# open-flash/swf-renderer

Measured on AMD Instinct MI355X. Metric: Mpixels/sec rasterized @ 4K, 10k-edge synthetic shape set, higher is better.
Workload: dtype i32+f64(exact integers)/u8

## Files before the change

### swf_renderer_amd/csrc/device_types.hpp

```cpp
#pragma once

#include <stdint.h>

#include "../../include/swfr.h"

namespace swfr {

constexpr int TILE_W = 64;
constexpr int TILE_H = 16;
constexpr int STRIP_H = 8;
constexpr int STRIPS_PER_TILE = TILE_H / STRIP_H;

struct DevEdge {
    int32_t ytop, ybot;
    int32_t x1, y1;
    int32_t dir;
    int32_t pad;
    int64_t ex;
    int64_t dy;
    int64_t dq, dr;
    double inv_dy;
    double inv_dx;
    int64_t fr;
    int64_t r15;
// ... 124 lines not shown
struct StripDesc {
    uint32_t wg;
    uint32_t band_begin, n_b;
    uint32_t pad;
};

struct StripTop {
    uint32_t any, pad;
    unsigned long long cover;
};
static_assert(sizeof(StripTop) == 16, "StripTop layout");

constexpr uint32_t XCDS = 8;
inline uint32_t strip_slots(uint32_t local_tile_rows, uint32_t strips_per_row) { return XCDS * ((local_tile_rows + XCDS - 1) / XCDS) * strips_per_row; }
constexpr uint32_t BIN_THREADS_LARGE = 1024, BIN_THREADS_SMALL = 256, BIN_SMALL_PATHS = 16 * BIN_THREADS_SMALL;

struct Frame2 {
    const swfr_edge* raw; const DevPath* paths;
    const swfr_style* styles;
    Sources src;
    const uint32_t* path_chunks; const uint32_t* path_slots; const uint32_t* path_inc;
    const uint32_t* band_off;
    const uint32_t* path_bands;
    ChunkInfo* chunks; BandSlot* band_slots; StripDesc* strips;
    uint32_t* strip_cost;
    DevEdge* edges; BandEntry2* band_list; uint8_t* cls; RowInfo2* rows; Cell* cells; SlowRow* slow; SlowRow* huge; uint32_t* counters;
    uint32_t* path_flag; uint32_t* path_queue;
    uint32_t* fb;
    StripTop* strip_top;
    uint32_t n_edges, n_paths, n_chunks, n_bands, n_strips, cell_slice, slow_cap;
// ... 17 lines not shown
```

### swf_renderer_amd/csrc/frame_layout.hpp

```cpp
#pragma once
#include <stddef.h>
#include <stdint.h>

#include "device_types.hpp"

namespace swfr {

inline size_t pad256(size_t bytes) { return (bytes + 255) & ~size_t(255); }

struct FrameDims {
    size_t n_edges = 0, n_paths = 0, n_slots = 0, n_rows = 0, n_chunks = 0, n_strips = 0, n_strip_slots = 0, cell_total = 0;
    template <class Layout>
    static FrameDims of_layout(const Layout& L, size_t n_edges, size_t n_paths) {
        return FrameDims{n_edges, n_paths, L.n_slots, L.n_rows, L.n_chunks, L.n_strips, L.n_strip_slots, L.cell_total};
    }

    size_t edge_count() const { return 2 * n_edges + 1; }
    size_t band_entry_count() const { return n_slots; }
    size_t row_count() const { return n_slots * TILE_H + 64; }
    size_t cell_count() const { return cell_total; }
    size_t slow_count() const { return 2 * (n_rows + 64); }
    size_t path_word_count() const { return n_paths + 64; }
    size_t chunk_count() const { return n_chunks + 1; }
    size_t band_slot_count() const { return n_slots + 8; }
    size_t strip_count() const { return n_strip_slots + 1; }
    size_t strip_cost_count() const { return n_strips + 1; }
};

template <class V>
void for_each_frame_buffer(Frame2& f, const FrameDims& d, V&& v) {
    v(f.edges, d.edge_count()); v(f.band_list, d.band_entry_count()); v(f.rows, d.row_count()); v(f.cells, d.cell_count());
    v(f.slow, d.slow_count()); v(f.huge, d.slow_count()); v(f.path_flag, d.path_word_count()); v(f.path_queue, d.path_word_count());
    v(f.chunks, d.chunk_count()); v(f.band_slots, d.band_slot_count()); v(f.strips, d.strip_count()); v(f.strip_cost, d.strip_cost_count());
    v(f.counters, size_t(C2_WORDS));
}
inline uint8_t* carve_frame(Frame2& f, const FrameDims& d, uint8_t* base) {
    for_each_frame_buffer(f, d, [&](auto*& p, size_t n) { p = reinterpret_cast<decltype(p + 0)>(base); base += pad256(n * sizeof(*p)); });
    return base;
}
inline size_t frame_work_bytes(const FrameDims& d) {
    Frame2 f{};
    size_t bytes = 0;
    for_each_frame_buffer(f, d, [&](auto* p, size_t n) { bytes += pad256(n * sizeof(*p)); });
    return bytes;
}

inline size_t cls_bytes_of(size_t n_slots, size_t tiles_x) { return (size_t(STRIPS_PER_TILE) * n_slots * tiles_x + 64 + 15) & ~size_t(15); }
inline size_t cls_region_bytes(size_t n_slots, size_t tiles_x, size_t n_strips) { return cls_bytes_of(n_slots, tiles_x) + (n_strips + 1) * sizeof(StripTop); }
inline size_t cls_region_bytes(const FrameDims& d, size_t tiles_x) { return cls_region_bytes(d.n_slots, tiles_x, d.n_strips); }
inline void set_cls_region(Frame2& f, const FrameDims& d, size_t tiles_x, uint8_t* base) {
    f.cls = base;
    f.strip_top = reinterpret_cast<StripTop*>(base + cls_bytes_of(d.n_slots, tiles_x));
}

}
```

### swf_renderer_amd/csrc/raster2.hip

```cpp
#include "raster_common.hip"

namespace swfr {

__device__ __forceinline__ void lds_barrier() {
#ifdef SWFR_EMU
    __syncthreads();
#else
    __builtin_amdgcn_fence(__ATOMIC_RELEASE, "workgroup", "local");
    __builtin_amdgcn_s_barrier();
    __builtin_amdgcn_fence(__ATOMIC_ACQUIRE, "workgroup", "local");
#endif
}

#ifdef SWFR_EMU
typedef const Frame2* FramePtr;
#define FRAME_PTR(frames, i) ((frames) + (i))
#else
typedef const Frame2 __attribute__((address_space(4)))* FramePtr;
#define FRAME_PTR(frames, i) ((FramePtr)((frames) + (i)))
#endif

#ifdef SWFR_TSTATS
#define TRACE_WGS 32768
__device__ uint32_t swfr_trace_buf[3][TRACE_WGS][8];
// ... 279 lines not shown
        for (uint32_t c = 0; c < nc; ++c) write_chunk(ip, c, a0, c0, inc0, slots0, first_edge, n_path_edges, band0);
    for (unsigned long long big = __ballot(nc > OWN_CHUNKS); big; big &= big - 1ull) {
        const int src = __ffsll((long long)big) - 1;
        const uint32_t b_nc = (uint32_t)__shfl((int)nc, src), b_path = (uint32_t)__shfl((int)ip, src), b_a0 = (uint32_t)__shfl((int)a0, src);
        const uint32_t b_c0 = (uint32_t)__shfl((int)c0, src), b_inc0 = (uint32_t)__shfl((int)inc0, src), b_slots0 = (uint32_t)__shfl((int)slots0, src);
        const uint32_t b_fe = (uint32_t)__shfl((int)first_edge, src), b_ne = (uint32_t)__shfl((int)n_path_edges, src), b_band0 = (uint32_t)__shfl((int)band0, src);
        for (uint32_t c = (uint32_t)lane; c < b_nc; c += 64u) write_chunk(b_path, c, b_a0, b_c0, b_inc0, b_slots0, b_fe, b_ne, b_band0);
    }
}
constexpr uint32_t ORDER_RANGES = 8;
__device__ __forceinline__ uint32_t order_range(uint32_t cost) {
    return cost >= 48u ? 0u : cost >= 32u ? 1u : cost >= 24u ? 2u : cost >= 16u ? 3u : cost >= 8u ? 4u : cost >= 4u ? 5u : cost >= 1u ? 6u : 7u;
}
constexpr uint32_t ORDER_U = 16;
template <uint32_t BIN_THREADS> __device__ __forceinline__ void order_body(FramePtr F, uint32_t x) {
    __shared__ uint2 rowinfo[256];
    __shared__ uint32_t cnt[ORDER_RANGES][ORDER_U][BIN_THREADS / 64];
    const int tid = threadIdx.x, lane = tid & 63, wave = tid >> 6;
    const uint32_t n_strips = F->n_strips, bc = F->band_stride, bi = F->band_first;
    const uint32_t per_row = STRIPS_PER_TILE * (uint32_t)F->tiles_x;
    const uint32_t n_local = n_strips / per_row;
    const uint32_t rows_x = (n_local + XCDS - 1 - x) / XCDS, max_rows = (n_local + XCDS - 1) / XCDS;
    const uint32_t n_mine = rows_x * per_row;
    const bool by_cost = F->strip_order != 0u;
    for (uint32_t j = (uint32_t)tid; j < rows_x && j < 256u; j += BIN_THREADS) {
        const uint32_t trow = (x + j * XCDS) * bc + bi, b0 = F->band_off[trow];
        rowinfo[j] = make_uint2(b0, F->band_off[trow + 1] - b0);
    }
    if (rows_x < max_rows)
        for (uint32_t j = (uint32_t)tid; j < per_row; j += BIN_THREADS) {
            StripDesc sd; sd.wg = ~0u; sd.band_begin = 0; sd.n_b = 0; sd.pad = 0;
            F->strips[(size_t)(n_mine + j) * XCDS + x] = sd;
        }
    __syncthreads();
    const uint32_t dq = BIN_THREADS / per_row, dr = BIN_THREADS - dq * per_row;
    auto advance = [&](uint32_t& j, uint32_t& pos) { j += dq; pos += dr; if (pos >= per_row) { pos -= per_row; ++j; } };
    auto strip_at = [&](uint32_t j, uint32_t pos) { return (x + j * XCDS) * per_row + pos; };
    for (uint32_t base = 0; base < n_mine; base += ORDER_U * BIN_THREADS) {
        const uint32_t n_round = min(n_mine - base, ORDER_U * BIN_THREADS), U = (n_round + BIN_THREADS - 1) / BIN_THREADS;
        unsigned long long ranges = 0;
// ... 42 lines not shown
            }
            __syncthreads();
        } else {
#pragma unroll
            for (uint32_t u = 0; u < ORDER_U; ++u) behind[u] = 0;
        }
        uint32_t j = j0, pos = pos0;
#pragma unroll
        for (uint32_t u = 0; u < ORDER_U; ++u) {
            if (u >= U) continue;
            const uint32_t i = base + u * BIN_THREADS + (uint32_t)tid;
            if (i < n_mine) {
                uint32_t rank = i;
                if (by_cost) rank = base + cnt[(uint32_t)(ranges >> (3 * u)) & 7u][u][wave] + behind[u];
                uint2 ri;
                if (j < 256u) ri = rowinfo[j]; else { const uint32_t trow = (x + j * XCDS) * bc + bi, b0 = F->band_off[trow]; ri = make_uint2(b0, F->band_off[trow + 1] - b0); }
                StripDesc sd; sd.wg = strip_at(j, pos); sd.band_begin = ri.x; sd.n_b = ri.y; sd.pad = (pos / STRIPS_PER_TILE) | ((x + j * XCDS) << 16);
                F->strips[(size_t)rank * XCDS + x] = sd;
            }
            advance(j, pos);
        }
        __syncthreads();
    }
}
__global__ __launch_bounds__(1024) __attribute__((amdgpu_num_sgpr(80))) void k2_bin_b(const Frame2* __restrict__ frames, uint32_t slow_kernels) { TRACE_DECL; TRACE_NOWAIT(0); bin_body<BIN_THREADS_LARGE, BIN_ORDER_FIRST_LARGE != 0>(FRAME_PTR(frames, blockIdx.y), slow_kernels); TRACE(7); TRACE_OUT(0, blockIdx.x); }
__global__ __launch_bounds__(256) void k2_bin_small_b(const Frame2* __restrict__ frames, uint32_t slow_kernels) { TRACE_DECL; TRACE_NOWAIT(0); bin_body<BIN_THREADS_SMALL, BIN_ORDER_FIRST_SMALL != 0>(FRAME_PTR(frames, blockIdx.y), slow_kernels); TRACE(7); TRACE_OUT(0, blockIdx.x); }

__device__ __forceinline__ uint32_t pack_sub_cell(int x, int sgn, int xminp, int xmaxp) {
    int col = x >> 8, f = x & 255, live = 1;
    if (col >= xmaxp) { col = xmaxp - 1; f = 0; live = 0; }
    else if (col < xminp) { col = xminp; f = 0; }
// ... 7 lines not shown
#define R2_WAVES 5
#endif
#define R2_ATTR __attribute__((amdgpu_waves_per_eu(R2_WAVES)))
#ifndef R2_WIDE_WAVES
#define R2_WIDE_WAVES 3
#endif
__global__ __launch_bounds__(64) R2_ATTR void k2_rows_b(const Frame2* __restrict__ frames) {
    FramePtr FR = FRAME_PTR(frames, blockIdx.y);
    if (blockIdx.x >= FR->n_chunks) return;
    rows3_chunk_body<ROWS_STAGE, ROWS_FAST_N>(FR, blockIdx.x);
}
__global__ __launch_bounds__(64) __attribute__((amdgpu_waves_per_eu(R2_WIDE_WAVES))) void k2_rows_wide_b(const Frame2* __restrict__ frames) {
    FramePtr FR = FRAME_PTR(frames, blockIdx.y);
    if (blockIdx.x >= FR->n_chunks) return;
    rows3_chunk_body<ROWS_STAGE_WIDE, ROWS_FAST_WIDE>(FR, blockIdx.x);
}

#include "mono.hip"

__global__ __launch_bounds__(64) void k2_rows_mono_b(const Frame2* __restrict__ frames) {
    FramePtr FR = FRAME_PTR(frames, blockIdx.y);
    if (blockIdx.x >= FR->n_chunks) return;
    mono_chunk_body(FR, blockIdx.x);
}
__global__ __launch_bounds__(HUGE_THREADS) void k2_rows_mono_huge_b(const Frame2* __restrict__ frames) { mono_huge_loop(FRAME_PTR(frames, blockIdx.y)); }


__device__ __forceinline__ void sort_pairs(uint16_t* __restrict__ dst, const int* __restrict__ cell, int p, int cnt) {
    const int x = 2 * p, y = 2 * p + 1;
    if (y < cnt) { const bool keep = cell[x] <= cell[y]; dst[x] = (uint16_t)(keep ? x : y); dst[y] = (uint16_t)(keep ? y : x); }
// ... 1314 lines not shown
#endif
__global__ __launch_bounds__(64) __attribute__((amdgpu_waves_per_eu(T2_WAVES_SHADED))) void k2_tiles_bitmap_b(const Frame2* __restrict__ frames, uint32_t* fb_to) { tiles3_body<1>(FRAME_PTR(frames, blockIdx.y), fb_to); }
__global__ __launch_bounds__(64) __attribute__((amdgpu_waves_per_eu(T2_WAVES_SHADED))) void k2_tiles_shaded_b(const Frame2* __restrict__ frames, uint32_t* fb_to) { tiles3_body<2>(FRAME_PTR(frames, blockIdx.y), fb_to); }
__global__ __launch_bounds__(64) __attribute__((amdgpu_waves_per_eu(T2_WAVES_BLEND))) void k2_tiles_blend_b(const Frame2* __restrict__ frames, uint32_t* fb_to) { tiles3_body<3>(FRAME_PTR(frames, blockIdx.y), fb_to); }
__global__ __launch_bounds__(64) __attribute__((amdgpu_waves_per_eu(T2_WAVES_LAYER))) void k2_tiles_layer_b(const Frame2* __restrict__ frames, uint32_t* fb_to) { tiles3_body<4>(FRAME_PTR(frames, blockIdx.y), fb_to); }
__global__ __launch_bounds__(64) __attribute__((amdgpu_waves_per_eu(T2_WAVES_LAYER))) void k2_tiles_mask_b(const Frame2* __restrict__ frames, uint32_t* fb_to) { tiles3_body<5>(FRAME_PTR(frames, blockIdx.y), fb_to); }
__global__ __launch_bounds__(64) __attribute__((amdgpu_waves_per_eu(T2_WAVES_LAYER))) void k2_tiles_fade_b(const Frame2* __restrict__ frames, uint32_t* fb_to) { tiles3_body<6>(FRAME_PTR(frames, blockIdx.y), fb_to); }
__global__ __launch_bounds__(64) __attribute__((amdgpu_waves_per_eu(T2_WAVES_LAYER))) void k2_tiles_alpha_b(const Frame2* __restrict__ frames, uint32_t* fb_to) { tiles3_body<7>(FRAME_PTR(frames, blockIdx.y), fb_to); }

void launch2_bin(hipStream_t st, const Frame2* frames, uint32_t n_frames, uint32_t max_edges, uint32_t max_paths, uint32_t max_bands, uint32_t slow_kernels, bool mono, uint32_t bin_threads) {
    const uint32_t T = bin_threads == BIN_THREADS_SMALL ? BIN_THREADS_SMALL : BIN_THREADS_LARGE;
    const uint32_t g = XCDS + max_bands + (mono ? 0u : (max_edges + T - 1) / T) + (max_paths + T - 1) / T;
    if (T == BIN_THREADS_SMALL) hipLaunchKernelGGL(k2_bin_small_b, dim3(g, n_frames), dim3(BIN_THREADS_SMALL), 0, st, frames, slow_kernels);
    else hipLaunchKernelGGL(k2_bin_b, dim3(g, n_frames), dim3(BIN_THREADS_LARGE), 0, st, frames, slow_kernels);
}
void launch2_rows(hipStream_t st, const Frame2* frames, uint32_t n_frames, uint32_t max_chunks, uint32_t max_path_edges, bool wide, bool mono) {
    if (!max_chunks) return;
    if (mono) { hipLaunchKernelGGL(k2_rows_mono_b, dim3(max_chunks, n_frames), dim3(64), 0, st, frames); return; }
    if (wide || max_path_edges > ROWS_STAGE) hipLaunchKernelGGL(k2_rows_wide_b, dim3(max_chunks, n_frames), dim3(64), 0, st, frames);
    else hipLaunchKernelGGL(k2_rows_b, dim3(max_chunks, n_frames), dim3(64), 0, st, frames);
}
void launch2_rows_slow(hipStream_t st, const Frame2* frames, uint32_t n_frames, uint32_t grid_slow, uint32_t grid_huge, uint32_t max_passes, bool mono) {
    if (mono) { hipLaunchKernelGGL(k2_rows_mono_huge_b, dim3(grid_huge ? grid_huge : 64u, n_frames), dim3(HUGE_THREADS), 0, st, frames); return; }
    if (grid_slow) hipLaunchKernelGGL(k2_start_ranks_b, dim3(grid_slow / 4 + 1, n_frames), dim3(256), 0, st, frames);
    for (uint32_t pass = 0; pass < SLOW_PASSES; ++pass) {
        if (grid_slow) hipLaunchKernelGGL(k2_rows_slow_b, dim3(grid_slow, n_frames), dim3(64), 0, st, frames, pass);
        if (grid_huge) hipLaunchKernelGGL(k2_rows_huge_b, dim3(grid_huge, n_frames), dim3(HUGE_THREADS), 0, st, frames, pass);
        if (pass + 1 >= max_passes) break;
    }
}
__device__ __forceinline__ void linear_pieces_body(FramePtr FR) {
    if (blockIdx.x >= FR->n_linear_records) return;
    const DevGradient* G = FR->src.gradients + blockIdx.x;
    if (G->pad <= 0) return;
    int32_t* table = const_cast<int32_t*>(FR->src.fparams) + (G->pad - 1);
// ... 85 lines not shown
```

### swf_renderer_amd/csrc/renderer.cpp

```cpp
#include <hip/hip_runtime.h>

#include <algorithm>
#include <chrono>
#include <cfloat>
#include <cmath>
#include <cstdio>
#include <cstdlib>
#include <cstring>
#include <exception>
#include <map>
#include <memory>
#include <stdexcept>
#include <string>
#include <unordered_map>
#include <vector>

#include "../../include/swfr.h"
#include "device_types.hpp"
#include "frame_layout.hpp"
#include "frame_builder.hpp"
#include "shape_decoder.hpp"
#include "bitmap_decode.hpp"

namespace swfr {
void launch2_bin(hipStream_t, const Frame2*, uint32_t, uint32_t, uint32_t, uint32_t, uint32_t, bool, uint32_t);
void launch2_rows(hipStream_t, const Frame2*, uint32_t, uint32_t, uint32_t, bool, bool);
void launch2_rows_slow(hipStream_t, const Frame2*, uint32_t, uint32_t, uint32_t, uint32_t, bool);
void launch2_tiles(hipStream_t, const Frame2*, uint32_t, uint32_t, uint32_t, int, uint32_t*);
void launch2_linear_pieces(hipStream_t, const Frame2*, uint32_t, uint32_t);
void launch_unpremultiply(hipStream_t, const uint32_t*, uint32_t*, size_t);
void launch_pack_band(hipStream_t, const uint32_t*, uint32_t*, int, int, uint32_t, uint32_t, uint32_t);
void launch_cxform_texels(hipStream_t, const uint8_t*, uint32_t*, size_t, const uint32_t*);
void launch_blur_capture(hipStream_t, const uint32_t*, uint32_t*, size_t);
void launch_blur_pass(hipStream_t, const uint32_t*, uint32_t*, uint32_t, uint32_t, uint32_t, bool);
void launch_shadow_alpha(hipStream_t, const uint32_t*, uint32_t*, uint32_t, uint32_t, int32_t, int32_t);
void launch_shadow_finish(hipStream_t, const uint32_t*, const uint32_t*, bool, uint32_t*, size_t, uint32_t, uint32_t, uint32_t);
}

using namespace swfr;

namespace {
// ... 119 lines not shown
    swfr_config cfg{};
    bool has_device = false;
    std::string error;
    std::unique_ptr<FrameBuilder> builder;
    std::string json_scratch;

    hipStream_t stream = nullptr;
    uint32_t* h_counters = nullptr;
    std::vector<hipEvent_t> ev;
    struct Scene {
        SceneArena arena;
        FrameDims dims;
        LaunchPlan bounds{};
        Frame2 proto{};
        Frame2* frames_dev = nullptr;
        uint32_t slow_passes = SLOW_PASSES;
        bool slow_verified = false;
        int slow_state = 0;
    };
    Scene scn[4];
    struct FrameSet {
        hipStream_t stream = nullptr;
        DevBuf<uint8_t> work, cls;
        DevBuf<uint32_t> strip_cost;
        uint32_t* counters = nullptr;
        DevBuf<uint32_t> d_fb;
        hipGraph_t graph = nullptr;
        hipGraphExec_t graph_exec = nullptr;
        uint64_t graph_key = 0;
    };
    FrameSet fs[4];
    uint64_t scene_gen = 0;
    int resident_batch = 2;
#ifdef SWFR_EMU
    int use_graphs = 0;
#else
    int use_graphs = 0;
#endif
    DevBuf<DevBitmap> d_bitmap_table;
// ... 17 lines not shown
    DevBuf<uint32_t> shadow_scratch;
    std::vector<DevBitmap> blur_table;
    bool bitmap_table_dirty = false, bitmap_table_dirty_copied = false;
    bool scene_ready = false, fb_valid = false;
    swfr_timing timing{};
    swfr_path_timing path_timing{};
    int force_chunk_rows = 0;
    int strip_order = 1;
    int event_stride = 16;
    bool event_stride_given = false;
    bool mono = false;
    int fast_limit = 16;
    int tiles_grid = 0;
    int bin_threads = 0;
    uint32_t last_bin_threads = 0;
    int tiles_shaders = 0;
    bool rows_wide = false;
    struct BatchGroup {
        SceneArena arena;
        DevBuf<uint8_t> work, cls;
        hipStream_t stream = nullptr;
        uint32_t* h_counters = nullptr;
        size_t h_counters_cap = 0;
        hipEvent_t ev_begin = nullptr, ev_end = nullptr;
    };
    BatchGroup groups[2];
    int batch_frames = 64;
    uint32_t* targets[4] = {nullptr, nullptr, nullptr, nullptr};
    swfr_stats stats = {};
    DevBuf<uint8_t> rb_work, rb_cls;
// ... 5 lines not shown
    bool read_pending = false;
    uint32_t n_targets = 0, async_next = 0, async_used = 0;

    ~swfr_renderer() {
        if (has_device) {
            (void)hipSetDevice(cfg.device);
            d_bitmap_table.release(); d_tmp.release(); d_counters.release();
            rb_work.release(); rb_cls.release(); rb_frames.release(); rb_fb.release();
            for (auto& t : blur_tex) t.release();
            blur_scratch.release(); shadow_scratch.release();
            for (auto& e : rb_ev) if (e) (void)hipEventDestroy(e);
            if (h_image) (void)hipHostFree(h_image);
            if (read_done) (void)hipEventDestroy(read_done);
            for (int k = 0; k < 4; ++k) {
                FrameSet& x = fs[k];
                x.work.release(); x.cls.release(); x.strip_cost.release(); x.d_fb.release();
                if (x.graph_exec) (void)hipGraphExecDestroy(x.graph_exec);
                if (x.graph) (void)hipGraphDestroy(x.graph);
                if (k > 0 && x.stream) (void)hipStreamDestroy(x.stream);
                scn[k].arena.release();
            }
            if (h_counters) (void)hipHostFree(h_counters);
            for (auto& g : groups) {
                g.arena.release(); g.work.release(); g.cls.release();
                if (g.stream) (void)hipStreamDestroy(g.stream);
                if (g.h_counters) (void)hipHostFree(g.h_counters);
                if (g.ev_begin) { (void)hipEventDestroy(g.ev_begin); (void)hipEventDestroy(g.ev_end); }
            }
            for (auto& kv : bitmaps) {
                if (kv.second.pixels) (void)hipFree(kv.second.pixels);
                if (kv.second.d_straight) (void)hipFree(kv.second.d_straight);
// ... 814 lines not shown
    p.max_chunks = uint32_t(L.n_chunks); p.max_path_edges = L.max_path_edges; p.rows_wide = L.rows_wide;
    p.linear_grid = L.n_linear ? uint32_t(L.gradients.size()) : 0u;
    p.max_strips = uint32_t(L.n_strip_slots); p.shader_level = L.shader_level;
    return p;
}
void merge_bounds(LaunchPlan& p, const LaunchPlan& q) {
    p.max_edges = std::max(p.max_edges, q.max_edges); p.max_paths = std::max(p.max_paths, q.max_paths); p.max_bands = std::max(p.max_bands, q.max_bands);
    p.max_chunks = std::max(p.max_chunks, q.max_chunks); p.max_path_edges = std::max(p.max_path_edges, q.max_path_edges); p.rows_wide = p.rows_wide || q.rows_wide;
    p.linear_grid = std::max(p.linear_grid, q.linear_grid); p.max_strips = std::max(p.max_strips, q.max_strips); p.shader_level = std::max(p.shader_level, q.shader_level);
}
void place_frame(Frame2& f, const FrameDims& d, size_t tiles_x, uint8_t*& w, uint8_t*& c) {
    w = carve_frame(f, d, w);
    set_cls_region(f, d, tiles_x, c);
    c += pad256(cls_region_bytes(d, tiles_x));
}

int upload2(swfr_renderer* r, int si, bool all_sets, SceneView sv, uint32_t* fb_override, bool edges_tagged) {
    swfr_renderer::Scene& sc = r->scn[si];
    if (si == 0) r->scene_ready = false;
    if (r->async_used) {
        for (int k = 0; k < 4; ++k) if (r->fs[k].stream) HIP_CHECK(hipStreamSynchronize(r->fs[k].stream));
    }
    sc.slow_verified = false;
    sc.slow_state = si == 0 ? r->hint_slow_state : 0; sc.slow_passes = si == 0 ? r->hint_slow_passes : SLOW_PASSES;
    if (si > 0 && !r->fs[si].stream) HIP_CHECK(hipStreamCreateWithFlags(&r->fs[si].stream, hipStreamNonBlocking));
    const hipStream_t up_stream = r->fs[si].stream;
    const uint32_t tiles_x = (r->width + TILE_W - 1) / TILE_W;
    std::vector<swfr_edge> tagged;
    if (!edges_tagged) {
        tagged.assign(sv.edges, sv.edges + sv.n_edges);
        for (size_t i = 0; i < sv.n_paths; ++i)
            for (uint32_t k = 0; k < sv.paths[i].n_edges; ++k) tagged[sv.paths[i].first_edge + k].reserved = int32_t(i);
        if (r->mono)
            for (size_t i = 0; i < sv.n_paths; ++i)
                if (sv.paths[i].kind == SWFR_PATH_BOXES)
                    for (uint32_t k = 0; k < sv.paths[i].n_edges; ++k) round_box_to_pixels(tagged[sv.paths[i].first_edge + k]);
        sv.edges = tagged.data();
    }
    static thread_local FrameScratch scratch;
    static thread_local SceneLayout L;
    const SceneView a = prepare_frame(r, sv, up_stream, si == 0, scratch, L);
    const FrameDims dims = sc.dims = FrameDims::of_layout(L, a.n_edges, a.n_paths);
    sc.bounds = plan_bounds(L, a.n_edges, a.n_paths);
    SceneArena& A = sc.arena;
    A.begin(scene_arena_bytes(L, a) + SceneArena::padded(4 * sizeof(Frame2)) + 4096);
    Frame2 proto;
    std::memset(&proto, 0, sizeof proto);
    push_scene(A, L, a, proto);
    fill_frame_sizes(r, L, a, proto);
    if (r->bitmap_table_dirty) r->d_bitmap_table.reserve(r->bitmap_table.size());
    proto.src.bitmaps = r->d_bitmap_table.ptr;
    sc.proto = proto;
    const size_t cls_bytes = cls_region_bytes(dims, tiles_x);
    const int n_sets = std::max(1, std::min(r->in_flight, 4));
    Frame2 fr[4];
    std::memset(fr, 0, sizeof fr);
    for (int k = 0; k < 4; ++k) {
        if (all_sets ? k >= n_sets : k != si) continue;
        auto& x = r->fs[k];
        Frame2& f = fr[k];
        f = proto;
        if (!x.stream) HIP_CHECK(hipStreamCreateWithFlags(&x.stream, hipStreamNonBlocking));
        x.work.reserve(frame_work_bytes(dims)); x.cls.reserve(cls_bytes);
        uint8_t *w = x.work.ptr, *c = x.cls.ptr;
        place_frame(f, dims, tiles_x, w, c);
        const uint32_t* cost_before = x.strip_cost.ptr;
        x.strip_cost.reserve(dims.strip_cost_count());
        if (x.strip_cost.ptr != cost_before) HIP_CHECK(hipMemsetAsync(x.strip_cost.ptr, 0, x.strip_cost.cap * sizeof(uint32_t), up_stream));
        f.strip_cost = x.strip_cost.ptr;
        r->d_counters.reserve(4 * COUNTER_WORDS);
        f.counters = x.counters = r->d_counters.ptr + size_t(k) * COUNTER_WORDS;
        HIP_CHECK(hipMemsetAsync(x.cls.ptr, 0, cls_bytes, up_stream));
        if (!x.d_fb.ptr && !r->n_targets) {
            x.d_fb.reserve(size_t(r->width) * r->height);
            HIP_CHECK(hipMemsetAsync(x.d_fb.ptr, 0, size_t(r->width) * r->height * 4, up_stream));
        }
        f.fb = (fb_override && k == si) ? fb_override : (r->n_targets ? r->targets[uint32_t(k) % r->n_targets] : x.d_fb.ptr);
    }
    sc.frames_dev = static_cast<Frame2*>(A.push(fr, sizeof fr));
    A.flush(up_stream, si == 0);
    if (all_sets) {
        for (int k = 0; k < n_sets; ++k)
            if (k != si && r->fs[k].stream) HIP_CHECK(hipStreamWaitEvent(r->fs[k].stream, A.copied, 0));
    }
    if (r->bitmap_table_dirty) {
        if (!r->bitmap_table.empty())
            HIP_CHECK(hipMemcpyAsync(r->d_bitmap_table.ptr, r->bitmap_table.data(), r->bitmap_table.size() * sizeof(DevBitmap),
                                     hipMemcpyHostToDevice, r->stream));
        r->bitmap_table_dirty = false;
        r->bitmap_table_dirty_copied = true;
    }
    if (r->bitmap_table_dirty_copied) { HIP_CHECK(hipStreamSynchronize(r->stream)); r->bitmap_table_dirty_copied = false; }
    if (si == 0) { r->scene_ready = true; r->sets_ready = all_sets ? uint32_t(n_sets) : 1u; r->scene_from_builder = edges_tagged; ++r->scene_gen; }
    return SWFR_OK;
// ... 194 lines not shown
    }
    hipEvent_t ev_begin = r->ev[size_t(n_timed) * 4], ev_end = r->ev[size_t(n_timed) * 4 + 1];
    hipEvent_t* ev_join = &r->ev[size_t(n_timed) * 4 + 2];
    if (frames > 1 && r->use_graphs && sc.slow_verified && !(r->resident_batch >= 2 && stride > frames))
        for (uint32_t k = 0; k < n_sets; ++k) ensure_frame_graph(r, sc, r->fs[k]);
    HIP_CHECK(hipEventRecord(ev_begin, r->stream));
    order_frames_behind_pending_read(r);
#ifdef SWFR_BEGIN_WAIT
    for (uint32_t k = 1; k < n_sets; ++k) HIP_CHECK(hipStreamWaitEvent(r->fs[k].stream, ev_begin, 0));
#endif
    uint32_t rb = (r->resident_batch >= 2 && stride > frames) ? uint32_t(r->resident_batch) : 1u;
    while (rb > 1 && (rb > n_sets || n_sets % rb != 0)) --rb;
    const bool batched = rb > 1 && frames >= 2;
    uint32_t last_set = (frames - 1) % n_sets;
    int64_t last_on[4] = {-1, -1, -1, -1};
    if (batched) {
        const uint32_t groups = n_sets / rb;
        const LaunchPlan plan = plan_of(r, sc);
        uint32_t gi = 0;
        for (uint32_t f = 0; f < frames; f += rb, ++gi) {
            const uint32_t g = gi % groups, cnt = std::min(rb, frames - f);
            launch_chain(r, r->fs[g * rb].stream, sc.frames_dev + g * rb, cnt, plan, nullptr, nullptr);
            last_set = g * rb + cnt - 1;
            last_on[g * rb] = int64_t(gi);
        }
    }
    for (uint32_t f = 0; f < frames && !batched; ++f) {
        swfr_renderer::FrameSet& F = r->fs[f % n_sets];
        const bool timed = f >= first_timed && (f - first_timed) % stride == 0;
        if (!timed && frames > 1 && r->use_graphs && sc.slow_verified) launch_frame_graph(r, sc, F);
        else launch_frame(r, sc, F, nullptr, timed ? &r->ev[size_t((f - first_timed) / stride) * 4] : nullptr, n_sets > 1 && frames > 1);
        last_on[f % n_sets] = int64_t(f);
    }
    for (uint32_t k = 1; k < n_sets; ++k) {
        if (last_on[k] < 0) continue;
        HIP_CHECK(hipEventRecord(ev_join[k - 1], r->fs[k].stream));
        HIP_CHECK(hipStreamWaitEvent(r->stream, ev_join[k - 1], 0));
    }
    HIP_CHECK(hipEventRecord(ev_end, r->stream));
    HIP_CHECK(hipGetLastError());
    if (!r->h_counters) HIP_CHECK(hipHostMalloc(reinterpret_cast<void**>(&r->h_counters), 4 * COUNTER_WORDS * sizeof(uint32_t), hipHostMallocDefault));
    const uint32_t used_sets = std::min(frames, n_sets);
    HIP_CHECK(hipMemcpyAsync(r->h_counters, r->d_counters.ptr, size_t(used_sets) * COUNTER_WORDS * sizeof(uint32_t), hipMemcpyDeviceToHost, r->stream));
    for (;;) {
        int pick = -1;
        for (uint32_t k = 1; k < n_sets; ++k)
            if (last_on[k] >= 0 && (pick < 0 || last_on[k] < last_on[pick])) pick = int(k);
        if (pick < 0) break;
        if (r->fs[pick].stream) HIP_CHECK(hipStreamSynchronize(r->fs[pick].stream));
        last_on[pick] = -1;
    }
    HIP_CHECK(hipStreamSynchronize(r->stream));
    r->fb_cur = r->n_targets ? r->targets[last_set % r->n_targets] : r->fs[last_set].d_fb.ptr;
    uint32_t timed_frames = 0;
    for (uint32_t f = batched ? frames : first_timed; f < frames; f += stride, ++timed_frames) {
        hipEvent_t* e = &r->ev[size_t(timed_frames) * 4];
        float a = 0, b = 0, c = 0;
        HIP_CHECK(hipEventElapsedTime(&a, e[0], e[1]));
        HIP_CHECK(hipEventElapsedTime(&b, e[1], e[2]));
        HIP_CHECK(hipEventElapsedTime(&c, e[2], e[3]));
        setup_ms += a; rows_ms += b; tiles_ms += c;
    }
    HIP_CHECK(hipEventElapsedTime(&total_ms, ev_begin, ev_end));
    std::memcpy(counters, r->h_counters, sizeof counters);
    for (uint32_t k = 1; k < used_sets; ++k)
        for (uint32_t w : {uint32_t(C2_ERROR), uint32_t(C2_TIE_PAIRTEST_SKIPPED), uint32_t(C2_TIE_SORT_OVERFLOW), uint32_t(C2_TIE_DEPTH)})
            counters[w] |= r->h_counters[k * COUNTER_WORDS + w];
    r->timing = swfr_timing{total_ms, setup_ms, rows_ms, tiles_ms, frames, sc.dims.n_edges, sc.dims.n_paths, sc.dims.n_rows, 0, timed_frames};
    r->fb_valid = true;
    {
        uint32_t slow = 0, huge = 0;
        for (uint32_t k = 0; k < used_sets; ++k) { slow |= r->h_counters[k * COUNTER_WORDS + C2_SLOW]; huge |= r->h_counters[k * COUNTER_WORDS + C2_HUGE]; }
        uint32_t passes = 1;
        for (uint32_t k = 0; k < used_sets; ++k)
            for (uint32_t q = 1; q < SLOW_PASSES; ++q) {
                const uint32_t* c = r->h_counters + k * COUNTER_WORDS;
                if (c[C2_SLOWQ + q] | c[C2_HUGEQ + q]) { passes = std::max(passes, q + 1); huge |= c[C2_HUGEQ + q]; }
            }
// ... 385 lines not shown
    if (const char* fl = std::getenv("SWFR_FAST_LIMIT")) r->fast_limit = std::atoi(fl);
    if (const char* tg = std::getenv("SWFR_TILES_GRID")) r->tiles_grid = std::atoi(tg);
    if (const char* bt = std::getenv("SWFR_BIN_THREADS")) { const int v = std::atoi(bt); r->bin_threads = v == int(BIN_THREADS_SMALL) || v == int(BIN_THREADS_LARGE) ? v : 0; }
    if (const char* ts = std::getenv("SWFR_TILES_SHADERS")) r->tiles_shaders = std::min(std::max(std::atoi(ts), 0), 7);
    if (const char* rw = std::getenv("SWFR_ROWS_WIDE")) r->rows_wide = std::atoi(rw) != 0;
    if (const char* bf = std::getenv("SWFR_BATCH_FRAMES")) r->batch_frames = std::max(1, std::atoi(bf));
    if (const char* cr = std::getenv("SWFR_CHUNK_ROWS")) r->force_chunk_rows = std::atoi(cr);
    if (const char* so = std::getenv("SWFR_STRIP_ORDER")) r->strip_order = std::atoi(so);
    if (const char* fi = std::getenv("SWFR_FRAMES_IN_FLIGHT")) r->in_flight = std::atoi(fi);
    if (const char* es = std::getenv("SWFR_EVENT_STRIDE")) { r->event_stride = std::atoi(es); r->event_stride_given = true; }
    if (const char* ug = std::getenv("SWFR_GRAPHS")) r->use_graphs = std::atoi(ug);
#ifdef SWFR_EMU
    r->use_graphs = 0;
#endif
    if (const char* rb = std::getenv("SWFR_RESIDENT_BATCH")) r->resident_batch = std::atoi(rb);
    if (const char* cm = std::getenv("SWFR_CXFORM_CACHE_MB")) r->cx_budget = size_t(std::max(0, std::atoi(cm))) << 20;
    if (r->cfg.device == SWFR_DEVICE_HOST_ONLY) {
        *out = r.release();
        return SWFR_OK;
    }
    int count = 0;
    if (hipGetDeviceCount(&count) != hipSuccess || count <= 0) return SWFR_ERR_NO_DEVICE;
    if (r->cfg.device < 0 || r->cfg.device >= count) return SWFR_ERR_NO_DEVICE;
    r->has_device = true;
    swfr_renderer* raw = r.get();
    const int rc = guarded(raw, [&]() {
        HIP_CHECK(hipStreamCreateWithFlags(&raw->stream, hipStreamNonBlocking));
        raw->fs[0].stream = raw->stream;
        for (int k = 1; k < std::max(1, std::min(raw->in_flight, 4)); ++k) HIP_CHECK(hipStreamCreateWithFlags(&raw->fs[k].stream, hipStreamNonBlocking));
        for (int i = 0; i < 4 * 32 + 5; ++i) { hipEvent_t e = nullptr; HIP_CHECK(hipEventCreate(&e)); raw->ev.push_back(e); }
        raw->fs[0].d_fb.reserve(size_t(width) * height);
        HIP_CHECK(hipMemsetAsync(raw->fs[0].d_fb.ptr, 0, size_t(width) * height * 4, raw->stream));
        raw->d_counters.reserve(4 * COUNTER_WORDS);
        raw->fs[0].counters = raw->d_counters.ptr;
        HIP_CHECK(hipStreamSynchronize(raw->stream));
        return int(SWFR_OK);
    });
    if (rc != SWFR_OK) return rc;
    *out = r.release();
    return SWFR_OK;
}

void swfr_destroy(swfr_renderer* r) { delete r; }

int swfr_register_shape(swfr_renderer* r, const swfr_define_shape* tag, uint32_t* out_id) {
    if (!r || !tag || !out_id) return fail(r, SWFR_ERR_INVALID, "null argument");
    return guarded(r, [&]() {
        *out_id = r->builder->add_shape(decode_shape(*tag, false));
// ... 559 lines not shown
    return SWFR_OK;
}

int swfr_get_stats(swfr_renderer* r, swfr_stats* out) {
    if (!r || !out) return SWFR_ERR_INVALID;
    *out = r->stats;
    return SWFR_OK;
}

void* swfr_stream_handle(swfr_renderer* r, uint32_t set) { return (r && r->has_device && set < 4) ? static_cast<void*>(r->fs[set].stream) : nullptr; }

int swfr_wait(swfr_renderer* r) {
    if (!r) return SWFR_ERR_INVALID;
    if (!r->has_device) return fail(r, SWFR_ERR_NO_DEVICE, "host-only handle");
    return guarded(r, [&]() {
        if (!r->h_counters) HIP_CHECK(hipHostMalloc(reinterpret_cast<void**>(&r->h_counters), 4 * COUNTER_WORDS * sizeof(uint32_t), hipHostMallocDefault));
        int rc = SWFR_OK;
        for (uint32_t k = 0; k < 4; ++k) {
            if (!r->fs[k].stream || !r->fs[k].counters) continue;
            if (!(r->async_used >> k & 1u)) { HIP_CHECK(hipStreamSynchronize(r->fs[k].stream)); continue; }
            HIP_CHECK(hipMemcpyAsync(r->h_counters + k * COUNTER_WORDS, r->fs[k].counters, COUNTER_WORDS * sizeof(uint32_t), hipMemcpyDeviceToHost, r->fs[k].stream));
            HIP_CHECK(hipStreamSynchronize(r->fs[k].stream));
            if (rc == SWFR_OK) rc = check_counters(r, r->h_counters + k * COUNTER_WORDS);
        }
        r->async_used = 0;
        r->fb_valid = rc == SWFR_OK;
        return rc;
    });
}

long swfr_debug_copy(swfr_renderer* r, int what, void* dst, size_t bytes) {
    if (!r || !dst) return -long(SWFR_ERR_INVALID);
    if (!r->has_device) return -long(SWFR_ERR_NO_DEVICE);
    if (what == 2) {
        if (bytes < sizeof(uint32_t)) return 0;
        std::memcpy(dst, &r->last_bin_threads, sizeof(uint32_t));
        return long(sizeof(uint32_t));
    }
    if (!r->fs[0].work.ptr) return 0;
    const FrameDims& d = r->scn[0].dims;
    Frame2 f{};
    carve_frame(f, d, r->fs[0].work.ptr);
    const void* src = what == 0 ? static_cast<const void*>(f.rows) : static_cast<const void*>(f.cells);
    const size_t n = std::min(bytes, what == 0 ? d.row_count() * sizeof(RowInfo2) : d.cell_count() * sizeof(Cell));
    if (!n) return 0;
    if (hipDeviceSynchronize() != hipSuccess || hipMemcpy(dst, src, n, hipMemcpyDeviceToHost) != hipSuccess) return -long(SWFR_ERR_DEVICE);
    return long(n);
}

void* swfr_device_framebuffer(swfr_renderer* r) { return (r && r->has_device) ? (r->fb_cur ? r->fb_cur : r->fs[0].d_fb.ptr) : nullptr; }

// ... 3 lines not shown
```

Measured before the change: 375,700.

## Overlap next batch's binning with current rows kernel via double-buffered frames

Adds a second, parity-indexed set of per-frame buffers so the binning stage of the next batched launch can run inside the rows kernel of the current launch, using extra 64-thread blocks. This fused kernel (k2_rows_ahead_b) removes a separate bin launch and its serialization per batch in the resident-batch benchmark path. It costs extra memory for the duplicated buffers, more counter readback and parity bookkeeping, and bin work done with small 64-thread blocks that may be slower per item and compete with rows blocks for CUs.

```diff
diff --git a/swf_renderer_amd/csrc/device_types.hpp b/swf_renderer_amd/csrc/device_types.hpp
--- a/swf_renderer_amd/csrc/device_types.hpp
+++ b/swf_renderer_amd/csrc/device_types.hpp
@@ -162,6 +162,7 @@
 constexpr uint32_t XCDS = 8;
 inline uint32_t strip_slots(uint32_t local_tile_rows, uint32_t strips_per_row) { return XCDS * ((local_tile_rows + XCDS - 1) / XCDS) * strips_per_row; }
 constexpr uint32_t BIN_THREADS_LARGE = 1024, BIN_THREADS_SMALL = 256, BIN_SMALL_PATHS = 16 * BIN_THREADS_SMALL;
+constexpr uint32_t BIN_THREADS_AHEAD = 64;
 
 struct Frame2 {
     const swfr_edge* raw; const DevPath* paths;
diff --git a/swf_renderer_amd/csrc/frame_layout.hpp b/swf_renderer_amd/csrc/frame_layout.hpp
--- a/swf_renderer_amd/csrc/frame_layout.hpp
+++ b/swf_renderer_amd/csrc/frame_layout.hpp
@@ -28,11 +28,15 @@
 };
 
 template <class V>
+void for_each_frame_buffer_parity(Frame2& f, const FrameDims& d, V&& v) {
+    v(f.edges, d.edge_count(), true); v(f.band_list, d.band_entry_count(), true); v(f.rows, d.row_count(), false); v(f.cells, d.cell_count(), false);
+    v(f.slow, d.slow_count(), false); v(f.huge, d.slow_count(), false); v(f.path_flag, d.path_word_count(), true); v(f.path_queue, d.path_word_count(), false);
+    v(f.chunks, d.chunk_count(), true); v(f.band_slots, d.band_slot_count(), true); v(f.strips, d.strip_count(), true); v(f.strip_cost, d.strip_cost_count(), true);
+    v(f.counters, size_t(C2_WORDS), true);
+}
+template <class V>
 void for_each_frame_buffer(Frame2& f, const FrameDims& d, V&& v) {
-    v(f.edges, d.edge_count()); v(f.band_list, d.band_entry_count()); v(f.rows, d.row_count()); v(f.cells, d.cell_count());
-    v(f.slow, d.slow_count()); v(f.huge, d.slow_count()); v(f.path_flag, d.path_word_count()); v(f.path_queue, d.path_word_count());
-    v(f.chunks, d.chunk_count()); v(f.band_slots, d.band_slot_count()); v(f.strips, d.strip_count()); v(f.strip_cost, d.strip_cost_count());
-    v(f.counters, size_t(C2_WORDS));
+    for_each_frame_buffer_parity(f, d, [&](auto*& p, size_t n, bool) { v(p, n); });
 }
 inline uint8_t* carve_frame(Frame2& f, const FrameDims& d, uint8_t* base) {
     for_each_frame_buffer(f, d, [&](auto*& p, size_t n) { p = reinterpret_cast<decltype(p + 0)>(base); base += pad256(n * sizeof(*p)); });
@@ -45,6 +49,19 @@
     return bytes;
 }
 
+inline uint8_t* carve_frame_ahead(Frame2& f, const FrameDims& d, uint8_t* base) {
+    for_each_frame_buffer_parity(f, d, [&](auto*& p, size_t n, bool per_parity) {
+        if (per_parity) { p = reinterpret_cast<decltype(p + 0)>(base); base += pad256(n * sizeof(*p)); }
+    });
+    return base;
+}
+inline size_t frame_ahead_bytes(const FrameDims& d) {
+    Frame2 f{};
+    size_t bytes = 0;
+    for_each_frame_buffer_parity(f, d, [&](auto* p, size_t n, bool per_parity) { if (per_parity) bytes += pad256(n * sizeof(*p)); });
+    return bytes;
+}
+
 inline size_t cls_bytes_of(size_t n_slots, size_t tiles_x) { return (size_t(STRIPS_PER_TILE) * n_slots * tiles_x + 64 + 15) & ~size_t(15); }
 inline size_t cls_region_bytes(size_t n_slots, size_t tiles_x, size_t n_strips) { return cls_bytes_of(n_slots, tiles_x) + (n_strips + 1) * sizeof(StripTop); }
 inline size_t cls_region_bytes(const FrameDims& d, size_t tiles_x) { return cls_region_bytes(d.n_slots, tiles_x, d.n_strips); }
diff --git a/swf_renderer_amd/csrc/raster2.hip b/swf_renderer_amd/csrc/raster2.hip
--- a/swf_renderer_amd/csrc/raster2.hip
+++ b/swf_renderer_amd/csrc/raster2.hip
@@ -317,7 +317,8 @@
 }
 constexpr uint32_t ORDER_U = 16;
 template <uint32_t BIN_THREADS> __device__ __forceinline__ void order_body(FramePtr F, uint32_t x) {
-    __shared__ uint2 rowinfo[256];
+    constexpr uint32_t ROWINFO = BIN_THREADS >= BIN_THREADS_SMALL ? 256u : 32u;
+    __shared__ uint2 rowinfo[ROWINFO];
     __shared__ uint32_t cnt[ORDER_RANGES][ORDER_U][BIN_THREADS / 64];
     const int tid = threadIdx.x, lane = tid & 63, wave = tid >> 6;
     const uint32_t n_strips = F->n_strips, bc = F->band_stride, bi = F->band_first;
@@ -326,7 +327,7 @@
     const uint32_t rows_x = (n_local + XCDS - 1 - x) / XCDS, max_rows = (n_local + XCDS - 1) / XCDS;
     const uint32_t n_mine = rows_x * per_row;
     const bool by_cost = F->strip_order != 0u;
-    for (uint32_t j = (uint32_t)tid; j < rows_x && j < 256u; j += BIN_THREADS) {
+    for (uint32_t j = (uint32_t)tid; j < rows_x && j < ROWINFO; j += BIN_THREADS) {
         const uint32_t trow = (x + j * XCDS) * bc + bi, b0 = F->band_off[trow];
         rowinfo[j] = make_uint2(b0, F->band_off[trow + 1] - b0);
     }
@@ -399,7 +400,7 @@
                 uint32_t rank = i;
                 if (by_cost) rank = base + cnt[(uint32_t)(ranges >> (3 * u)) & 7u][u][wave] + behind[u];
                 uint2 ri;
-                if (j < 256u) ri = rowinfo[j]; else { const uint32_t trow = (x + j * XCDS) * bc + bi, b0 = F->band_off[trow]; ri = make_uint2(b0, F->band_off[trow + 1] - b0); }
+                if (j < ROWINFO) ri = rowinfo[j]; else { const uint32_t trow = (x + j * XCDS) * bc + bi, b0 = F->band_off[trow]; ri = make_uint2(b0, F->band_off[trow + 1] - b0); }
                 StripDesc sd; sd.wg = strip_at(j, pos); sd.band_begin = ri.x; sd.n_b = ri.y; sd.pad = (pos / STRIPS_PER_TILE) | ((x + j * XCDS) << 16);
                 F->strips[(size_t)rank * XCDS + x] = sd;
             }
@@ -437,6 +438,19 @@
     FramePtr FR = FRAME_PTR(frames, blockIdx.y);
     if (blockIdx.x >= FR->n_chunks) return;
     rows3_chunk_body<ROWS_STAGE_WIDE, ROWS_FAST_WIDE>(FR, blockIdx.x);
+}
+__global__ __launch_bounds__(64) R2_ATTR void k2_rows_ahead_b(const Frame2* __restrict__ frames, const Frame2* __restrict__ ahead, uint32_t n_ahead, uint32_t ahead_frames) {
+    if (blockIdx.x < n_ahead) {
+        if (blockIdx.y >= ahead_frames) return;
+        TRACE_DECL; TRACE_NOWAIT(0);
+        bin_body<BIN_THREADS_AHEAD, true>(FRAME_PTR(ahead, blockIdx.y), 0u);
+        TRACE(7); TRACE_OUT(0, blockIdx.x);
+        return;
+    }
+    FramePtr FR = FRAME_PTR(frames, blockIdx.y);
+    const uint32_t chunk = blockIdx.x - n_ahead;
+    if (chunk >= FR->n_chunks) return;
+    rows3_chunk_body<ROWS_STAGE, ROWS_FAST_N>(FR, chunk);
 }
 
 #include "mono.hip"
@@ -1781,11 +1795,17 @@
     if (T == BIN_THREADS_SMALL) hipLaunchKernelGGL(k2_bin_small_b, dim3(g, n_frames), dim3(BIN_THREADS_SMALL), 0, st, frames, slow_kernels);
     else hipLaunchKernelGGL(k2_bin_b, dim3(g, n_frames), dim3(BIN_THREADS_LARGE), 0, st, frames, slow_kernels);
 }
+bool rows_wide_instance(uint32_t max_path_edges, bool wide) { return wide || max_path_edges > ROWS_STAGE; }
 void launch2_rows(hipStream_t st, const Frame2* frames, uint32_t n_frames, uint32_t max_chunks, uint32_t max_path_edges, bool wide, bool mono) {
     if (!max_chunks) return;
     if (mono) { hipLaunchKernelGGL(k2_rows_mono_b, dim3(max_chunks, n_frames), dim3(64), 0, st, frames); return; }
-    if (wide || max_path_edges > ROWS_STAGE) hipLaunchKernelGGL(k2_rows_wide_b, dim3(max_chunks, n_frames), dim3(64), 0, st, frames);
+    if (rows_wide_instance(max_path_edges, wide)) hipLaunchKernelGGL(k2_rows_wide_b, dim3(max_chunks, n_frames), dim3(64), 0, st, frames);
     else hipLaunchKernelGGL(k2_rows_b, dim3(max_chunks, n_frames), dim3(64), 0, st, frames);
+}
+void launch2_rows_ahead(hipStream_t st, const Frame2* frames, const Frame2* ahead, uint32_t n_frames, uint32_t ahead_frames, uint32_t max_edges, uint32_t max_paths, uint32_t max_bands, uint32_t max_chunks) {
+    constexpr uint32_t T = BIN_THREADS_AHEAD;
+    const uint32_t n_ahead = XCDS + max_bands + (max_edges + T - 1) / T + (max_paths + T - 1) / T;
+    hipLaunchKernelGGL(k2_rows_ahead_b, dim3(n_ahead + max_chunks, n_frames), dim3(64), 0, st, frames, ahead, n_ahead, ahead_frames);
 }
 void launch2_rows_slow(hipStream_t st, const Frame2* frames, uint32_t n_frames, uint32_t grid_slow, uint32_t grid_huge, uint32_t max_passes, bool mono) {
     if (mono) { hipLaunchKernelGGL(k2_rows_mono_huge_b, dim3(grid_huge ? grid_huge : 64u, n_frames), dim3(HUGE_THREADS), 0, st, frames); return; }
diff --git a/swf_renderer_amd/csrc/renderer.cpp b/swf_renderer_amd/csrc/renderer.cpp
--- a/swf_renderer_amd/csrc/renderer.cpp
+++ b/swf_renderer_amd/csrc/renderer.cpp
@@ -25,6 +25,8 @@
 namespace swfr {
 void launch2_bin(hipStream_t, const Frame2*, uint32_t, uint32_t, uint32_t, uint32_t, uint32_t, bool, uint32_t);
 void launch2_rows(hipStream_t, const Frame2*, uint32_t, uint32_t, uint32_t, bool, bool);
+bool rows_wide_instance(uint32_t, bool);
+void launch2_rows_ahead(hipStream_t, const Frame2*, const Frame2*, uint32_t, uint32_t, uint32_t, uint32_t, uint32_t, uint32_t);
 void launch2_rows_slow(hipStream_t, const Frame2*, uint32_t, uint32_t, uint32_t, uint32_t, bool);
 void launch2_tiles(hipStream_t, const Frame2*, uint32_t, uint32_t, uint32_t, int, uint32_t*);
 void launch2_linear_pieces(hipStream_t, const Frame2*, uint32_t, uint32_t);
@@ -174,6 +176,7 @@
         LaunchPlan bounds{};
         Frame2 proto{};
         Frame2* frames_dev = nullptr;
+        Frame2* frames_ahead = nullptr;
         uint32_t slow_passes = SLOW_PASSES;
         bool slow_verified = false;
         int slow_state = 0;
@@ -183,6 +186,7 @@
         hipStream_t stream = nullptr;
         DevBuf<uint8_t> work, cls;
         DevBuf<uint32_t> strip_cost;
+        DevBuf<uint32_t> strip_cost_ahead;
         uint32_t* counters = nullptr;
         DevBuf<uint32_t> d_fb;
         hipGraph_t graph = nullptr;
@@ -230,6 +234,8 @@
     int tiles_grid = 0;
     int bin_threads = 0;
     uint32_t last_bin_threads = 0;
+    int bin_ahead = 1;
+    uint32_t last_ahead_launches = 0;
     int tiles_shaders = 0;
     bool rows_wide = false;
     struct BatchGroup {
@@ -265,7 +271,7 @@
             if (read_done) (void)hipEventDestroy(read_done);
             for (int k = 0; k < 4; ++k) {
                 FrameSet& x = fs[k];
-                x.work.release(); x.cls.release(); x.strip_cost.release(); x.d_fb.release();
+                x.work.release(); x.cls.release(); x.strip_cost.release(); x.strip_cost_ahead.release(); x.d_fb.release();
                 if (x.graph_exec) (void)hipGraphExecDestroy(x.graph_exec);
                 if (x.graph) (void)hipGraphDestroy(x.graph);
                 if (k > 0 && x.stream) (void)hipStreamDestroy(x.stream);
@@ -1110,6 +1116,11 @@
     set_cls_region(f, d, tiles_x, c);
     c += pad256(cls_region_bytes(d, tiles_x));
 }
+void place_frame_ahead(Frame2& f, const FrameDims& d, size_t tiles_x, uint8_t*& w, uint8_t*& c) {
+    w = carve_frame_ahead(f, d, w);
+    set_cls_region(f, d, tiles_x, c);
+    c += pad256(cls_region_bytes(d, tiles_x));
+}
 
 int upload2(swfr_renderer* r, int si, bool all_sets, SceneView sv, uint32_t* fb_override, bool edges_tagged) {
     swfr_renderer::Scene& sc = r->scn[si];
@@ -1139,7 +1150,7 @@
     const FrameDims dims = sc.dims = FrameDims::of_layout(L, a.n_edges, a.n_paths);
     sc.bounds = plan_bounds(L, a.n_edges, a.n_paths);
     SceneArena& A = sc.arena;
-    A.begin(scene_arena_bytes(L, a) + SceneArena::padded(4 * sizeof(Frame2)) + 4096);
+    A.begin(scene_arena_bytes(L, a) + SceneArena::padded(8 * sizeof(Frame2)) + 4096);
     Frame2 proto;
     std::memset(&proto, 0, sizeof proto);
     push_scene(A, L, a, proto);
@@ -1149,7 +1160,8 @@
     sc.proto = proto;
     const size_t cls_bytes = cls_region_bytes(dims, tiles_x);
     const int n_sets = std::max(1, std::min(r->in_flight, 4));
-    Frame2 fr[4];
+    const bool ahead = all_sets && r->bin_ahead && !r->mono && r->cfg.band_count <= 1;
+    Frame2 fr[8];
     std::memset(fr, 0, sizeof fr);
     for (int k = 0; k < 4; ++k) {
         if (all_sets ? k >= n_sets : k != si) continue;
@@ -1157,23 +1169,34 @@
         Frame2& f = fr[k];
         f = proto;
         if (!x.stream) HIP_CHECK(hipStreamCreateWithFlags(&x.stream, hipStreamNonBlocking));
-        x.work.reserve(frame_work_bytes(dims)); x.cls.reserve(cls_bytes);
+        x.work.reserve(frame_work_bytes(dims) + (ahead ? frame_ahead_bytes(dims) : 0)); x.cls.reserve(ahead ? pad256(cls_bytes) + cls_bytes : cls_bytes);
         uint8_t *w = x.work.ptr, *c = x.cls.ptr;
         place_frame(f, dims, tiles_x, w, c);
         const uint32_t* cost_before = x.strip_cost.ptr;
         x.strip_cost.reserve(dims.strip_cost_count());
         if (x.strip_cost.ptr != cost_before) HIP_CHECK(hipMemsetAsync(x.strip_cost.ptr, 0, x.strip_cost.cap * sizeof(uint32_t), up_stream));
         f.strip_cost = x.strip_cost.ptr;
-        r->d_counters.reserve(4 * COUNTER_WORDS);
+        r->d_counters.reserve(8 * COUNTER_WORDS);
         f.counters = x.counters = r->d_counters.ptr + size_t(k) * COUNTER_WORDS;
-        HIP_CHECK(hipMemsetAsync(x.cls.ptr, 0, cls_bytes, up_stream));
+        HIP_CHECK(hipMemsetAsync(x.cls.ptr, 0, ahead ? pad256(cls_bytes) + cls_bytes : cls_bytes, up_stream));
         if (!x.d_fb.ptr && !r->n_targets) {
             x.d_fb.reserve(size_t(r->width) * r->height);
             HIP_CHECK(hipMemsetAsync(x.d_fb.ptr, 0, size_t(r->width) * r->height * 4, up_stream));
         }
         f.fb = (fb_override && k == si) ? fb_override : (r->n_targets ? r->targets[uint32_t(k) % r->n_targets] : x.d_fb.ptr);
+        if (ahead) {
+            Frame2& f1 = fr[4 + k];
+            f1 = f;
+            place_frame_ahead(f1, dims, tiles_x, w, c);
+            const uint32_t* cost1_before = x.strip_cost_ahead.ptr;
+            x.strip_cost_ahead.reserve(dims.strip_cost_count());
+            if (x.strip_cost_ahead.ptr != cost1_before) HIP_CHECK(hipMemsetAsync(x.strip_cost_ahead.ptr, 0, x.strip_cost_ahead.cap * sizeof(uint32_t), up_stream));
+            f1.strip_cost = x.strip_cost_ahead.ptr;
+            f1.counters = r->d_counters.ptr + size_t(4 + k) * COUNTER_WORDS;
+        }
     }
     sc.frames_dev = static_cast<Frame2*>(A.push(fr, sizeof fr));
+    sc.frames_ahead = ahead ? sc.frames_dev + 4 : nullptr;
     A.flush(up_stream, si == 0);
     if (all_sets) {
         for (int k = 0; k < n_sets; ++k)
@@ -1398,13 +1421,35 @@
     const bool batched = rb > 1 && frames >= 2;
     uint32_t last_set = (frames - 1) % n_sets;
     int64_t last_on[4] = {-1, -1, -1, -1};
+    uint32_t last_parity[4] = {0, 0, 0, 0};
+    r->last_ahead_launches = 0;
     if (batched) {
         const uint32_t groups = n_sets / rb;
         const LaunchPlan plan = plan_of(r, sc);
+        const bool ahead = r->bin_ahead && sc.frames_ahead && sc.slow_verified && !plan.run_slow && !plan.linear_grid && !r->mono && !r->bin_threads &&
+                           !r->use_graphs && !rows_wide_instance(plan.max_path_edges, plan.rows_wide);
+        const uint32_t launches = (frames + rb - 1) / rb;
         uint32_t gi = 0;
         for (uint32_t f = 0; f < frames; f += rb, ++gi) {
             const uint32_t g = gi % groups, cnt = std::min(rb, frames - f);
-            launch_chain(r, r->fs[g * rb].stream, sc.frames_dev + g * rb, cnt, plan, nullptr, nullptr);
+            const hipStream_t st = r->fs[g * rb].stream;
+            if (!ahead) launch_chain(r, st, sc.frames_dev + g * rb, cnt, plan, nullptr, nullptr);
+            else {
+                const uint32_t parity = (gi / groups) & 1u;
+                const Frame2* cur = (parity ? sc.frames_ahead : sc.frames_dev) + g * rb;
+                const Frame2* next = (parity ? sc.frames_dev : sc.frames_ahead) + g * rb;
+                if (gi < groups) {
+                    r->last_bin_threads = plan.bin_threads;
+                    launch2_bin(st, cur, cnt, plan.max_edges, plan.max_paths, plan.max_bands, 0u, false, plan.bin_threads);
+                }
+                if (gi + groups < launches) {
+                    const uint32_t next_cnt = std::min(rb, frames - (f + groups * rb));
+                    launch2_rows_ahead(st, cur, next, cnt, next_cnt, plan.max_edges, plan.max_paths, plan.max_bands, plan.max_chunks);
+                    ++r->last_ahead_launches;
+                } else launch2_rows(st, cur, cnt, plan.max_chunks, plan.max_path_edges, false, false);
+                launch2_tiles(st, cur, cnt, plan.max_strips, plan.tiles_grid, plan.shader_level, nullptr);
+                for (uint32_t k = 0; k < cnt; ++k) last_parity[g * rb + k] = parity;
+            }
             last_set = g * rb + cnt - 1;
             last_on[g * rb] = int64_t(gi);
         }
@@ -1423,9 +1468,10 @@
     }
     HIP_CHECK(hipEventRecord(ev_end, r->stream));
     HIP_CHECK(hipGetLastError());
-    if (!r->h_counters) HIP_CHECK(hipHostMalloc(reinterpret_cast<void**>(&r->h_counters), 4 * COUNTER_WORDS * sizeof(uint32_t), hipHostMallocDefault));
+    if (!r->h_counters) HIP_CHECK(hipHostMalloc(reinterpret_cast<void**>(&r->h_counters), 8 * COUNTER_WORDS * sizeof(uint32_t), hipHostMallocDefault));
     const uint32_t used_sets = std::min(frames, n_sets);
-    HIP_CHECK(hipMemcpyAsync(r->h_counters, r->d_counters.ptr, size_t(used_sets) * COUNTER_WORDS * sizeof(uint32_t), hipMemcpyDeviceToHost, r->stream));
+    const bool any_ahead = r->last_ahead_launches != 0;
+    HIP_CHECK(hipMemcpyAsync(r->h_counters, r->d_counters.ptr, size_t(any_ahead ? 8 : used_sets) * COUNTER_WORDS * sizeof(uint32_t), hipMemcpyDeviceToHost, r->stream));
     for (;;) {
         int pick = -1;
         for (uint32_t k = 1; k < n_sets; ++k)
@@ -1446,6 +1492,8 @@
         setup_ms += a; rows_ms += b; tiles_ms += c;
     }
     HIP_CHECK(hipEventElapsedTime(&total_ms, ev_begin, ev_end));
+    for (uint32_t k = 0; k < used_sets; ++k)
+        if (last_parity[k]) std::memcpy(r->h_counters + k * COUNTER_WORDS, r->h_counters + (4 + k) * COUNTER_WORDS, COUNTER_WORDS * sizeof(uint32_t));
     std::memcpy(counters, r->h_counters, sizeof counters);
     for (uint32_t k = 1; k < used_sets; ++k)
         for (uint32_t w : {uint32_t(C2_ERROR), uint32_t(C2_TIE_PAIRTEST_SKIPPED), uint32_t(C2_TIE_SORT_OVERFLOW), uint32_t(C2_TIE_DEPTH)})
@@ -1861,6 +1909,7 @@
     r->use_graphs = 0;
 #endif
     if (const char* rb = std::getenv("SWFR_RESIDENT_BATCH")) r->resident_batch = std::atoi(rb);
+    if (const char* ba = std::getenv("SWFR_BIN_AHEAD")) r->bin_ahead = std::atoi(ba) != 0;
     if (const char* cm = std::getenv("SWFR_CXFORM_CACHE_MB")) r->cx_budget = size_t(std::max(0, std::atoi(cm))) << 20;
     if (r->cfg.device == SWFR_DEVICE_HOST_ONLY) {
         *out = r.release();
@@ -1878,7 +1927,7 @@
         for (int i = 0; i < 4 * 32 + 5; ++i) { hipEvent_t e = nullptr; HIP_CHECK(hipEventCreate(&e)); raw->ev.push_back(e); }
         raw->fs[0].d_fb.reserve(size_t(width) * height);
         HIP_CHECK(hipMemsetAsync(raw->fs[0].d_fb.ptr, 0, size_t(width) * height * 4, raw->stream));
-        raw->d_counters.reserve(4 * COUNTER_WORDS);
+        raw->d_counters.reserve(8 * COUNTER_WORDS);
         raw->fs[0].counters = raw->d_counters.ptr;
         HIP_CHECK(hipStreamSynchronize(raw->stream));
         return int(SWFR_OK);
@@ -2468,7 +2517,7 @@
     if (!r) return SWFR_ERR_INVALID;
     if (!r->has_device) return fail(r, SWFR_ERR_NO_DEVICE, "host-only handle");
     return guarded(r, [&]() {
-        if (!r->h_counters) HIP_CHECK(hipHostMalloc(reinterpret_cast<void**>(&r->h_counters), 4 * COUNTER_WORDS * sizeof(uint32_t), hipHostMallocDefault));
+        if (!r->h_counters) HIP_CHECK(hipHostMalloc(reinterpret_cast<void**>(&r->h_counters), 8 * COUNTER_WORDS * sizeof(uint32_t), hipHostMallocDefault));
         int rc = SWFR_OK;
         for (uint32_t k = 0; k < 4; ++k) {
             if (!r->fs[k].stream || !r->fs[k].counters) continue;
@@ -2489,6 +2538,11 @@
     if (what == 2) {
         if (bytes < sizeof(uint32_t)) return 0;
         std::memcpy(dst, &r->last_bin_threads, sizeof(uint32_t));
+        return long(sizeof(uint32_t));
+    }
+    if (what == 3) {
+        if (bytes < sizeof(uint32_t)) return 0;
+        std::memcpy(dst, &r->last_ahead_launches, sizeof(uint32_t));
         return long(sizeof(uint32_t));
     }
     if (!r->fs[0].work.ptr) return 0;
```

Result: faster. 408,700 (median of 6 runs) (+8.8%).
